# OpenImagingLab/AdaptiveISP

Measured on AMD Instinct MI355X. Metric: ISP+YOLO forward images/sec @1280x720 bs8, higher is better.
Workload: dtype bf16; 1 GPU; batch 8 x 1280x720 fp32 RGB, 5-step ISP schedule ['E', 'CCM', 'NLM', 'Shr', 'T'] (teacher-forced, policy/heads evaluated every step) + YOLOv3 forward @1280x736 bf16 (random-init weights); per_gpu_batch=8, global_batch=8, parallelism=replicas x1

## Files before the change

### adaptiveisp_amd/_lib.py

```python
import ctypes
import os

import numpy as np
import torch

_HERE = os.path.dirname(os.path.abspath(__file__))
LIB_PATH = os.environ.get("ADAISP_LIB") or os.path.join(_HERE, "csrc", "libadaisp.so")

OP_ZERO, OP_EXPOSURE, OP_GAMMA, OP_CCM, OP_SHARPEN, OP_NLM, OP_TONE = -1, 0, 1, 2, 3, 4, 5
OP_CONTRAST, OP_SATPLUS, OP_WNB, OP_WB, OP_USM, OP_SHARPEN_V2, OP_COLOR = 6, 7, 8, 9, 10, 11, 12
MAX_PARAMS = 24
CLIP01 = 1
NLM_EXACT = 2
NLM_SEP_V1 = 4
NO_USM = 8
NLM_TILE32 = 16
ABI_VERSION = 9
UNP_UNPROCESS = 1
UNP_NOISE = 2

EXPORTS = ("adaisp_forward", "adaisp_forward_uniform", "adaisp_process", "adaisp_backward_params", "adaisp_backward_image", "adaisp_backward_image_workspace_bytes", "adaisp_pool64", "adaisp_pool64_backward", "adaisp_demosaic", "adaisp_unprocess", "adaisp_unprocess_bayer", "adaisp_demosaic_rects", "adaisp_demosaic_ex", "adaisp_demosaic_rects_ex", "adaisp_resize_u8", "adaisp_raw_load", "adaisp_raw_correct", "adaisp_export_u8", "adaisp_nlm_general", "adaisp_nlm_general_workspace_bytes", "adaisp_num_params",
           "adaisp_policy_conv", "adaisp_policy_fc1", "adaisp_policy_finish",
           "adaisp_trunk_train_fwd", "adaisp_trunk_train_bwd", "adaisp_trunk_train_workspace_bytes", "adaisp_trunk_train_scratch_bytes",
           "adaisp_critic_planes_fwd", "adaisp_critic_planes_bwd", "adaisp_td_fwd", "adaisp_td_bwd",
           "adaisp_policy_tail_fwd", "adaisp_policy_tail_bwd", "adaisp_image_stats", "adaisp_clip_adam_step", "adaisp_clip_adam_step_dev", "adaisp_heads_fwd", "adaisp_heads_bwd",
           "adaisp_strerror", "adaisp_abi_version")

_lib = None


class AdaispError(RuntimeError):
    pass


def load():
    global _lib
    if _lib is not None:
        return _lib
    if not os.path.exists(LIB_PATH):
# ... 84 lines not shown


def _stream():
    return ctypes.c_void_p(torch.cuda.current_stream().cuda_stream)


def _img_shape(img):
    if img.dim() != 4 or img.shape[1] != 3:
        raise ValueError(f"expected a [B,3,H,W] image, got {tuple(img.shape)}")
    return int(img.shape[0]), int(img.shape[2]), int(img.shape[3])


def image_stats(img):
    L = load()
    img = _dev_f32(img.detach(), "img")
    B = int(img.shape[0])
    buf = torch.empty((B, 2 + 128), dtype=torch.float32, device=img.device)
    with torch.cuda.device(img.device):
        rc = L.adaisp_image_stats(img.data_ptr(), buf.data_ptr(), buf.data_ptr() + 8 * B, B, img.numel() // B, _stream())
    _check(rc, "adaisp_image_stats")
    return buf.view(-1)[:2 * B].view(B, 2)


def process(op, img, params, clip=False, out=None, nlm_exact=False, nlm_v1=False, nlm_tile32=False):
    L = load()
    img = _dev_f32(img, "img")
    B, H, W = _img_shape(img)
    params = _dev_f32(params.reshape(B, -1), "params")
    if out is None:
        out = torch.empty_like(img)
    with torch.cuda.device(img.device):
        rc = L.adaisp_process(int(op), img.data_ptr(), out.data_ptr(), params.data_ptr(), params.shape[1], B, H, W,
                              (CLIP01 if clip else 0) | (NLM_EXACT if nlm_exact else 0) | (NLM_SEP_V1 if nlm_v1 else 0) |
                              (NLM_TILE32 if nlm_tile32 else 0),
                              _stream())
    _check(rc, "adaisp_process")
    _wrote(out)
    return out


def forward(img, op_ids, params, clip=True, pooled=None, out=None, nlm_exact=False, no_usm=False, host_op=None):
    L = load()
    img = _dev_f32(img, "img")
    B, H, W = _img_shape(img)
    params = _dev_f32(params.reshape(B, -1), "params")
    if host_op is None:
        if op_ids.dtype != torch.int32 or not op_ids.is_cuda:
            raise TypeError("op_ids must be an int32 device tensor")
        op_ids = op_ids.contiguous()
    if pooled is not None and (tuple(pooled.shape) != (B, 3, 64, 64) or pooled.dtype != torch.float32 or
                               pooled.device != img.device or not pooled.is_contiguous()):
        raise ValueError(f"pooled must be a contiguous float32 [{B},3,64,64] tensor on {img.device}")
    if out is None:
        out = torch.empty_like(img)
    elif (out.shape != img.shape or out.dtype != torch.float32 or out.device != img.device or not out.is_contiguous()):
        raise ValueError(f"out must be a contiguous float32 {tuple(img.shape)} tensor on {img.device}, got {out.dtype} "
                         f"{tuple(out.shape)} on {out.device}")
    flags = (CLIP01 if clip else 0) | (NLM_EXACT if nlm_exact else 0) | (NO_USM if no_usm else 0)
    with torch.cuda.device(img.device):
        if host_op is not None:
            rc = L.adaisp_forward_uniform(int(host_op), img.data_ptr(), out.data_ptr(),
                                          pooled.data_ptr() if pooled is not None else None, params.data_ptr(),
                                          params.shape[1], B, H, W, flags, _stream())
        else:
            rc = L.adaisp_forward(img.data_ptr(), out.data_ptr(), pooled.data_ptr() if pooled is not None else None,
                                  op_ids.data_ptr(), params.data_ptr(), params.shape[1], B, H, W, flags, _stream())
    _check(rc, "adaisp_forward")
    _wrote(out)
    _wrote(pooled)
    return out


def nlm_general(img, h, search_window_size, patch_size, out=None):
    L = load()
    img = _dev_f32(img, "img")
    B, H, W = _img_shape(img)
    h = _dev_f32(h.reshape(B, -1), "h")
    if out is None:
        out = torch.empty_like(img)
    nbytes = int(L.adaisp_nlm_general_workspace_bytes(B, H, W))
    ws = torch.empty(nbytes // 4, dtype=torch.float32, device=img.device)
# ... 316 lines not shown
```

### adaptiveisp_amd/csrc/isp_nlm.hip

```cpp
#include "isp_filter_math.h"
#ifndef NLM_FMA
#define NLM_FMA 1
#endif
#ifndef NLM_ABL
#define NLM_ABL 0
#endif

namespace adaisp {
namespace {

constexpr int kThreads = 256;
constexpr int TW = 64, TH = 32, RPT = 8;
constexpr int SR = 5, PR = 2;
constexpr int HY = SR + PR;
constexpr int YP = TW + 2 * HY;
constexpr int YROWS = TH + 2 * HY;
constexpr int CP = TW + 2 * SR;
constexpr int CROWS = TH + 2 * SR;
constexpr int NK = RPT + 2 * PR;
constexpr int kYBytes = ((YROWS * YP * 8 + 15) / 16) * 16;
constexpr int kSmemBytes = kYBytes + 3 * CROWS * CP * 4;

typedef float v2f __attribute__((ext_vector_type(2)));

__device__ __forceinline__ v2f pk_sub_bcast_lo(v2f a, v2f b) {
    v2f d;
    asm("v_pk_add_f32 %0, %1, %2 op_sel_hi:[0,1] neg_lo:[0,1] neg_hi:[0,1]" : "=v"(d) : "v"(a), "v"(b));
    return d;
}
__device__ __forceinline__ v2f pk_sub_bcast_hi(v2f a, v2f b) {
    return v2f{a.y, a.y} - b;
}

template <bool GRAD>
__global__ __launch_bounds__(kThreads) void k_nlm(const float* __restrict__ img, float* __restrict__ out,
                                                  const int32_t* __restrict__ ids, int uniform_op,
                                                  const float* __restrict__ params, int pstride, int H, int W,
                                                  const float* __restrict__ grad_out, float* __restrict__ grad_params) {
    extern __shared__ __attribute__((aligned(16))) unsigned char nlm_smem[];
    v2f* ylds2 = reinterpret_cast<v2f*>(nlm_smem);
    float* clds = reinterpret_cast<float*>(nlm_smem + kYBytes);

    const int b = blockIdx.z;
    const int op = ids ? ids[b] : uniform_op;
    if (op != ADAISP_OP_NLM) return;
    const long plane = (long)H * W;
    const float* __restrict__ in = img + (long)b * 3 * plane;
    float* __restrict__ o = out + (long)b * 3 * plane;
    const int x0 = blockIdx.x * TW, y0 = blockIdx.y * TH;
    const int tid = threadIdx.x;
// ... 284 lines not shown
        if (mine && params[(long)b * pstride] > 0.0f) {
#pragma unroll
            for (int r = 0; r < RPT; ++r) {
                const int gy = y0 + rb + r;
                if (gy < H) {
                    const long g = (long)gy * W + gx;
#pragma unroll
                    for (int c = 0; c < 3; ++c) {
                        const float oc = num[c][r] / den[r];
                        if (oc >= 0.0f && oc <= 1.0f) acc += go[g + c * plane] * (ga[c][r] - oc * gb[r]) / den[r];
                    }
                }
            }
        }
        __shared__ float red[4];
#pragma unroll
        for (int off = 32; off > 0; off >>= 1) acc += __shfl_xor(acc, off, 64);
        if ((tid & 63) == 0) red[tid >> 6] = acc;
        __syncthreads();
        if (tid == 0) atomicAdd(grad_params + (long)b * pstride, (red[0] + red[1]) + (red[2] + red[3]));
    }
}

template <int RQ>
__global__ __launch_bounds__(kThreads) void k_nlm_fwd(const float* __restrict__ img, float* __restrict__ out,
                                                      const int32_t* __restrict__ ids, int uniform_op,
                                                      const float* __restrict__ params, int pstride, int H, int W) {
    constexpr int TH = 8 * RQ, HALF = TH / 2;
    constexpr int YROWS = TH + 2 * HY, CROWS = TH + 2 * SR;
    constexpr int Y2ROWS = YROWS - HALF;
    constexpr int B2ROWS = CROWS - HALF;
    __shared__ v2f y2[Y2ROWS * SP];
    __shared__ v2f crg[CROWS * SP];
    __shared__ v2f cb2[B2ROWS * SP];
    const int b = blockIdx.z;
    const int op = ids ? ids[b] : uniform_op;
    if (op != ADAISP_OP_NLM) return;
    const long plane = (long)H * W;
    const float* __restrict__ in = img + (long)b * 3 * plane;
    const int x0 = blockIdx.x * SW, y0 = blockIdx.y * TH;
    const int tid = threadIdx.x;

    float* y2f = reinterpret_cast<float*>(y2);
    float* cb2f = reinterpret_cast<float*>(cb2);
    for (int q0 = tid; q0 < YROWS * SP; q0 += 4 * kThreads) {
        float rr[4], gg4[4], bb4[4];
#pragma unroll
// ... 16 lines not shown
            const int cy = ly - PR;
            if (cy >= 0 && cy < CROWS) {
                crg[cy * SP + lx] = v2f{r, gg};
                if (cy < B2ROWS) cb2f[(cy * SP + lx) * 2] = bb;
                if (cy >= HALF) cb2f[((cy - HALF) * SP + lx) * 2 + 1] = bb;
            }
        }
    }
    __syncthreads();

    const int lane = tid & 63, ty = tid >> 6;
    const int rb = ty * RQ;
    const float hh = fmaxf(params[(long)b * pstride], 0.0f) + 1e-8f;
    const float nc = -1.44269504088896341f / hh;

    v2f yc2[RQ + 2 * PR];
#pragma unroll
    for (int j = 0; j < RQ + 2 * PR; ++j) yc2[j] = y2[(rb + HY - PR + j) * SP + lane + SR];

    v2f nrgA[RQ], nrgB[RQ], nb2[RQ], den2[RQ];
#pragma unroll
    for (int i = 0; i < RQ; ++i) nrgA[i] = nrgB[i] = nb2[i] = den2[i] = v2f{0.0f, 0.0f};

    for (int dx = -SR; dx <= SR; ++dx) {
        for (int dy = -SR; dy <= SR; ++dy) {
            const v2f* ys = y2 + (rb + HY - PR - dy) * SP + lane + SR - dx;
            float c[2 * RQ];
#if NLM_FMA
            v2f dd[RQ + 2 * PR];
#pragma unroll
            for (int j = 0; j < RQ + 2 * PR; ++j) dd[j] = yc2[j] - ys[j * SP];
#pragma unroll
            for (int i = 0; i < RQ; ++i) {
                v2f cc = dd[i + 4] * dd[i + 4];
                cc = __builtin_elementwise_fma(dd[i + 3], dd[i + 3], cc);
                cc = __builtin_elementwise_fma(dd[i + 2], dd[i + 2], cc);
                cc = __builtin_elementwise_fma(dd[i + 1], dd[i + 1], cc);
                cc = __builtin_elementwise_fma(dd[i], dd[i], cc);
                c[2 * i] = cc.x;
                c[2 * i + 1] = cc.y;
            }
#else
            v2f S[RQ + 2 * PR];
#pragma unroll
            for (int j = 0; j < RQ + 2 * PR; ++j) {
                const v2f d = yc2[j] - ys[j * SP];
                S[j] = d * d;
            }
#pragma unroll
            for (int i = 0; i < RQ; ++i) {
                const v2f cc = (((S[i + 4] + S[i + 3]) + S[i + 2]) + S[i + 1]) + S[i];
                c[2 * i] = cc.x;
                c[2 * i + 1] = cc.y;
            }
#endif
            float D[2 * RQ], t1[2 * RQ], t2[2 * RQ], P[2 * RQ];
#if NLM_ABL == 2
#pragma unroll
            for (int i = 0; i < 2 * RQ; ++i) D[i] = c[i];
            if (false)
#endif
            if constexpr (RQ == 4) {
                asm("s_nop 1\n\t"
                    "v_add_f32_dpp %8, %32, %32 wave_shl:1 row_mask:0xf bank_mask:0xf bound_ctrl:0\n\t"
                    "v_add_f32_dpp %9, %33, %33 wave_shl:1 row_mask:0xf bank_mask:0xf bound_ctrl:0\n\t"
                    "v_add_f32_dpp %10, %34, %34 wave_shl:1 row_mask:0xf bank_mask:0xf bound_ctrl:0\n\t"
                    "v_add_f32_dpp %11, %35, %35 wave_shl:1 row_mask:0xf bank_mask:0xf bound_ctrl:0\n\t"
                    "v_add_f32_dpp %12, %36, %36 wave_shl:1 row_mask:0xf bank_mask:0xf bound_ctrl:0\n\t"
                    "v_add_f32_dpp %13, %37, %37 wave_shl:1 row_mask:0xf bank_mask:0xf bound_ctrl:0\n\t"
                    "v_add_f32_dpp %14, %38, %38 wave_shl:1 row_mask:0xf bank_mask:0xf bound_ctrl:0\n\t"
                    "v_add_f32_dpp %15, %39, %39 wave_shl:1 row_mask:0xf bank_mask:0xf bound_ctrl:0\n\t"
                    "v_add_f32_dpp %24, %32, %32 wave_shr:1 row_mask:0xf bank_mask:0xf bound_ctrl:0\n\t"
                    "v_add_f32_dpp %25, %33, %33 wave_shr:1 row_mask:0xf bank_mask:0xf bound_ctrl:0\n\t"
                    "v_add_f32_dpp %26, %34, %34 wave_shr:1 row_mask:0xf bank_mask:0xf bound_ctrl:0\n\t"
                    "v_add_f32_dpp %27, %35, %35 wave_shr:1 row_mask:0xf bank_mask:0xf bound_ctrl:0\n\t"
                    "v_add_f32_dpp %28, %36, %36 wave_shr:1 row_mask:0xf bank_mask:0xf bound_ctrl:0\n\t"
                    "v_add_f32_dpp %29, %37, %37 wave_shr:1 row_mask:0xf bank_mask:0xf bound_ctrl:0\n\t"
                    "v_add_f32_dpp %30, %38, %38 wave_shr:1 row_mask:0xf bank_mask:0xf bound_ctrl:0\n\t"
                    "v_add_f32_dpp %31, %39, %39 wave_shr:1 row_mask:0xf bank_mask:0xf bound_ctrl:0\n\t"
                    "v_add_f32_dpp %16, %8, %32 wave_shl:1 row_mask:0xf bank_mask:0xf bound_ctrl:0\n\t"
                    "v_add_f32_dpp %17, %9, %33 wave_shl:1 row_mask:0xf bank_mask:0xf bound_ctrl:0\n\t"
                    "v_add_f32_dpp %18, %10, %34 wave_shl:1 row_mask:0xf bank_mask:0xf bound_ctrl:0\n\t"
                    "v_add_f32_dpp %19, %11, %35 wave_shl:1 row_mask:0xf bank_mask:0xf bound_ctrl:0\n\t"
                    "v_add_f32_dpp %20, %12, %36 wave_shl:1 row_mask:0xf bank_mask:0xf bound_ctrl:0\n\t"
                    "v_add_f32_dpp %21, %13, %37 wave_shl:1 row_mask:0xf bank_mask:0xf bound_ctrl:0\n\t"
                    "v_add_f32_dpp %22, %14, %38 wave_shl:1 row_mask:0xf bank_mask:0xf bound_ctrl:0\n\t"
                    "v_add_f32_dpp %23, %15, %39 wave_shl:1 row_mask:0xf bank_mask:0xf bound_ctrl:0\n\t"
                    "v_add_f32_dpp %0, %24, %16 wave_shr:1 row_mask:0xf bank_mask:0xf bound_ctrl:0\n\t"
                    "v_add_f32_dpp %1, %25, %17 wave_shr:1 row_mask:0xf bank_mask:0xf bound_ctrl:0\n\t"
                    "v_add_f32_dpp %2, %26, %18 wave_shr:1 row_mask:0xf bank_mask:0xf bound_ctrl:0\n\t"
                    "v_add_f32_dpp %3, %27, %19 wave_shr:1 row_mask:0xf bank_mask:0xf bound_ctrl:0\n\t"
                    "v_add_f32_dpp %4, %28, %20 wave_shr:1 row_mask:0xf bank_mask:0xf bound_ctrl:0\n\t"
                    "v_add_f32_dpp %5, %29, %21 wave_shr:1 row_mask:0xf bank_mask:0xf bound_ctrl:0\n\t"
                    "v_add_f32_dpp %6, %30, %22 wave_shr:1 row_mask:0xf bank_mask:0xf bound_ctrl:0\n\t"
                    "v_add_f32_dpp %7, %31, %23 wave_shr:1 row_mask:0xf bank_mask:0xf bound_ctrl:0"
                    : "=&v"(D[0]), "=&v"(D[1]), "=&v"(D[2]), "=&v"(D[3]), "=&v"(D[4]), "=&v"(D[5]), "=&v"(D[6]), "=&v"(D[7]),
                      "=&v"(t1[0]), "=&v"(t1[1]), "=&v"(t1[2]), "=&v"(t1[3]), "=&v"(t1[4]), "=&v"(t1[5]), "=&v"(t1[6]), "=&v"(t1[7]),
                      "=&v"(t2[0]), "=&v"(t2[1]), "=&v"(t2[2]), "=&v"(t2[3]), "=&v"(t2[4]), "=&v"(t2[5]), "=&v"(t2[6]), "=&v"(t2[7]),
                      "=&v"(P[0]), "=&v"(P[1]), "=&v"(P[2]), "=&v"(P[3]), "=&v"(P[4]), "=&v"(P[5]), "=&v"(P[6]), "=&v"(P[7])
                    : "v"(c[0]), "v"(c[1]), "v"(c[2]), "v"(c[3]), "v"(c[4]), "v"(c[5]), "v"(c[6]), "v"(c[7]));
            } else {
                asm("s_nop 1\n\t"
                    "v_add_f32_dpp %6, %24, %24 wave_shl:1 row_mask:0xf bank_mask:0xf bound_ctrl:0\n\t"
                    "v_add_f32_dpp %7, %25, %25 wave_shl:1 row_mask:0xf bank_mask:0xf bound_ctrl:0\n\t"
                    "v_add_f32_dpp %8, %26, %26 wave_shl:1 row_mask:0xf bank_mask:0xf bound_ctrl:0\n\t"
                    "v_add_f32_dpp %9, %27, %27 wave_shl:1 row_mask:0xf bank_mask:0xf bound_ctrl:0\n\t"
                    "v_add_f32_dpp %10, %28, %28 wave_shl:1 row_mask:0xf bank_mask:0xf bound_ctrl:0\n\t"
                    "v_add_f32_dpp %11, %29, %29 wave_shl:1 row_mask:0xf bank_mask:0xf bound_ctrl:0\n\t"
                    "v_add_f32_dpp %18, %24, %24 wave_shr:1 row_mask:0xf bank_mask:0xf bound_ctrl:0\n\t"
                    "v_add_f32_dpp %19, %25, %25 wave_shr:1 row_mask:0xf bank_mask:0xf bound_ctrl:0\n\t"
                    "v_add_f32_dpp %20, %26, %26 wave_shr:1 row_mask:0xf bank_mask:0xf bound_ctrl:0\n\t"
                    "v_add_f32_dpp %21, %27, %27 wave_shr:1 row_mask:0xf bank_mask:0xf bound_ctrl:0\n\t"
                    "v_add_f32_dpp %22, %28, %28 wave_shr:1 row_mask:0xf bank_mask:0xf bound_ctrl:0\n\t"
                    "v_add_f32_dpp %23, %29, %29 wave_shr:1 row_mask:0xf bank_mask:0xf bound_ctrl:0\n\t"
                    "v_add_f32_dpp %12, %6, %24 wave_shl:1 row_mask:0xf bank_mask:0xf bound_ctrl:0\n\t"
                    "v_add_f32_dpp %13, %7, %25 wave_shl:1 row_mask:0xf bank_mask:0xf bound_ctrl:0\n\t"
                    "v_add_f32_dpp %14, %8, %26 wave_shl:1 row_mask:0xf bank_mask:0xf bound_ctrl:0\n\t"
                    "v_add_f32_dpp %15, %9, %27 wave_shl:1 row_mask:0xf bank_mask:0xf bound_ctrl:0\n\t"
                    "v_add_f32_dpp %16, %10, %28 wave_shl:1 row_mask:0xf bank_mask:0xf bound_ctrl:0\n\t"
                    "v_add_f32_dpp %17, %11, %29 wave_shl:1 row_mask:0xf bank_mask:0xf bound_ctrl:0\n\t"
                    "v_add_f32_dpp %0, %18, %12 wave_shr:1 row_mask:0xf bank_mask:0xf bound_ctrl:0\n\t"
                    "v_add_f32_dpp %1, %19, %13 wave_shr:1 row_mask:0xf bank_mask:0xf bound_ctrl:0\n\t"
                    "v_add_f32_dpp %2, %20, %14 wave_shr:1 row_mask:0xf bank_mask:0xf bound_ctrl:0\n\t"
                    "v_add_f32_dpp %3, %21, %15 wave_shr:1 row_mask:0xf bank_mask:0xf bound_ctrl:0\n\t"
                    "v_add_f32_dpp %4, %22, %16 wave_shr:1 row_mask:0xf bank_mask:0xf bound_ctrl:0\n\t"
                    "v_add_f32_dpp %5, %23, %17 wave_shr:1 row_mask:0xf bank_mask:0xf bound_ctrl:0"
                    : "=&v"(D[0]), "=&v"(D[1]), "=&v"(D[2]), "=&v"(D[3]), "=&v"(D[4]), "=&v"(D[5]),
                      "=&v"(t1[0]), "=&v"(t1[1]), "=&v"(t1[2]), "=&v"(t1[3]), "=&v"(t1[4]), "=&v"(t1[5]),
                      "=&v"(t2[0]), "=&v"(t2[1]), "=&v"(t2[2]), "=&v"(t2[3]), "=&v"(t2[4]), "=&v"(t2[5]),
                      "=&v"(P[0]), "=&v"(P[1]), "=&v"(P[2]), "=&v"(P[3]), "=&v"(P[4]), "=&v"(P[5])
                    : "v"(c[0]), "v"(c[1]), "v"(c[2]), "v"(c[3]), "v"(c[4]), "v"(c[5]));
            }
            const v2f* rg = crg + (rb + SR - dy) * SP + lane + SR - dx;
            const v2f* bl = cb2 + (rb + SR - dy) * SP + lane + SR - dx;
#pragma unroll
            for (int i = 0; i < RQ; ++i) {
#if NLM_ABL == 1
                const v2f wgt = v2f{D[2 * i], D[2 * i + 1]} * nc + 1.0f;
#elif NLM_ABL == 4
                const v2f ex = v2f{D[2 * i], D[2 * i + 1]} * nc;
                const v2f wgt = v2f{__builtin_amdgcn_exp2f(ex.x), __builtin_amdgcn_exp2f(ex.y)};
#else
                const v2f dist = v2f{__builtin_amdgcn_sqrtf(D[2 * i]), __builtin_amdgcn_sqrtf(D[2 * i + 1])};
                const v2f ex = dist * nc;
                const v2f wgt = v2f{__builtin_amdgcn_exp2f(ex.x), __builtin_amdgcn_exp2f(ex.y)};
#endif
#if NLM_ABL == 3
                den2[i] += wgt;
                continue;
#endif
                nrgA[i] = __builtin_elementwise_fma(rg[i * SP], v2f{wgt.x, wgt.x}, nrgA[i]);
                nrgB[i] = __builtin_elementwise_fma(rg[(i + HALF) * SP], v2f{wgt.y, wgt.y}, nrgB[i]);
                nb2[i] = __builtin_elementwise_fma(bl[i * SP], wgt, nb2[i]);
                den2[i] += wgt;
            }
        }
    }

    const int gx = x0 - 2 + lane;
    const bool mine = lane >= 2 && lane < 2 + SW && gx < W;
    float* __restrict__ o = out + (long)b * 3 * plane;
    if (mine) {
#pragma unroll
        for (int i = 0; i < RQ; ++i)
#pragma unroll
            for (int e = 0; e < 2; ++e) {
                const int gy = y0 + rb + i + e * HALF;
                if (gy < H) {
                    const long g = (long)gy * W + gx;
                    const float den = den2[i][e];
                    const v2f n2 = e ? nrgB[i] : nrgA[i];
                    o[g] = clamp01(n2.x / den);
                    o[g + plane] = clamp01(n2.y / den);
                    o[g + 2 * plane] = clamp01(nb2[i][e] / den);
                }
            }
    }
// ... 36 lines not shown
        }
    float* o = out + (long)b * 3 * plane + (long)yy * W + x;
    o[0] = clamp01(n0 / den); o[plane] = clamp01(n1 / den); o[2 * plane] = clamp01(n2 / den);
}

}

hipError_t launch_nlm_general(const float* img, float* out, const float* h, int hstride, float* workspace, int B, int H, int W,
                              int search, int patch, hipStream_t s) {
    const long plane = (long)H * W, total = plane * B;
    hipLaunchKernelGGL(k_nlm_luma, dim3((unsigned)((total + kThreads - 1) / kThreads)), dim3(kThreads), 0, s, img, workspace, plane, total);
    hipLaunchKernelGGL(k_nlm_general, dim3((W + 63) / 64, (H + 3) / 4, B), dim3(kThreads), 0, s, img, workspace, out, h, hstride, H, W,
                       search / 2, patch / 2);
    return hipGetLastError();
}

hipError_t launch_nlm(const Batch& a, hipStream_t s) {
    if (!(a.flags & ADAISP_NLM_EXACT)) {
        dim3 g((a.W + SW - 1) / SW, (a.H + TH - 1) / TH, a.B);
        if (a.flags & ADAISP_NLM_SEP_V1)
            hipLaunchKernelGGL(k_nlm_sep<false>, g, dim3(kThreads), 0, s, a.img, a.out, a.ids, a.uniform_op, a.params,
                               a.pstride, a.H, a.W, static_cast<const float*>(nullptr), static_cast<float*>(nullptr));
        else if (a.flags & ADAISP_NLM_TILE32)
            hipLaunchKernelGGL(k_nlm_fwd<4>, g, dim3(kThreads), 0, s, a.img, a.out, a.ids, a.uniform_op, a.params, a.pstride,
                               a.H, a.W);
        else
            hipLaunchKernelGGL(k_nlm_fwd<3>, dim3(g.x, (a.H + 23) / 24, a.B), dim3(kThreads), 0, s, a.img, a.out, a.ids,
                               a.uniform_op, a.params, a.pstride, a.H, a.W);
        return hipGetLastError();
    }
    dim3 grid((a.W + TW - 1) / TW, (a.H + TH - 1) / TH, a.B);
    static bool configured = false;
    if (!configured) {
        hipError_t e = hipFuncSetAttribute(reinterpret_cast<const void*>(k_nlm<false>),
                                           hipFuncAttributeMaxDynamicSharedMemorySize, kSmemBytes);
        if (e != hipSuccess) return e;
        configured = true;
    }
    hipLaunchKernelGGL(k_nlm<false>, grid, dim3(kThreads), kSmemBytes, s, a.img, a.out, a.ids, a.uniform_op, a.params, a.pstride,
                       a.H, a.W, static_cast<const float*>(nullptr), static_cast<float*>(nullptr));
    return hipGetLastError();
}

hipError_t launch_nlm_backward(const float* img, const float* grad_out, const int32_t* ids, const float* params,
                               int pstride, float* grad_params, int B, int H, int W, unsigned flags, hipStream_t s) {
    if (!(flags & ADAISP_NLM_EXACT)) {
        dim3 g((W + SW - 1) / SW, (H + TH - 1) / TH, B);
        hipLaunchKernelGGL(k_nlm_sep<true>, g, dim3(kThreads), 0, s, img, static_cast<float*>(nullptr), ids, 0, params,
                           pstride, H, W, grad_out, grad_params);
        return hipGetLastError();
    }
// ... 15 lines not shown
```

### include/adaisp.h

```cpp
#ifndef ADAISP_H_
#define ADAISP_H_

#include <stdint.h>

#ifdef __cplusplus
extern "C" {
#endif

#define ADAISP_ABI_VERSION 9

enum adaisp_op {
    ADAISP_OP_ZERO       = -1,
    ADAISP_OP_EXPOSURE   = 0,
    ADAISP_OP_GAMMA      = 1,
    ADAISP_OP_CCM        = 2,
    ADAISP_OP_SHARPEN    = 3,
    ADAISP_OP_NLM        = 4,
    ADAISP_OP_TONE       = 5,
    ADAISP_OP_CONTRAST   = 6,
    ADAISP_OP_SATPLUS    = 7,
    ADAISP_OP_WNB        = 8,
    ADAISP_OP_WB         = 9,
    ADAISP_OP_USM        = 10,
    ADAISP_OP_SHARPEN_V2 = 11,
    ADAISP_OP_COLOR      = 12,
    ADAISP_OP_COUNT      = 13
};

#define ADAISP_MAX_PARAMS 24

#define ADAISP_CLIP01 1u
#define ADAISP_NLM_EXACT 2u
#define ADAISP_NLM_SEP_V1 4u
#define ADAISP_NO_USM 8u
#define ADAISP_NLM_TILE32 16u

#define ADAISP_OK          0
#define ADAISP_EINVAL     -1
#define ADAISP_EOP        -2
#define ADAISP_EALIAS     -3
#define ADAISP_ESHAPE     -4
#define ADAISP_ELAUNCH    -5

int adaisp_forward(const float* img, float* out, float* pooled64_next,
                   const int32_t* filter_id, const float* params, int param_stride,
                   int B, int H, int W, unsigned flags, void* stream);

int adaisp_forward_uniform(int op, const float* img, float* out, float* pooled64_next,
                           const float* params, int param_stride,
                           int B, int H, int W, unsigned flags, void* stream);

int adaisp_process(int op, const float* img, float* out,
                   const float* params, int param_stride,
                   int B, int H, int W, unsigned flags, void* stream);

int adaisp_backward_params(const float* img, const float* grad_out,
                           const int32_t* filter_id, const float* params, int param_stride,
                           float* grad_params,
// ... 284 lines not shown
```

Before: 1975 images/sec.

## Software-pipeline NLM search loop with register sliding window across dy offsets

Refactors the NLM forward kernel's inner search loop into helper functions and adds a pipelined variant, used by default, for the 3-row-per-thread path. As dy advances, the variant slides guide and colour rows through registers, loading only one new row per step, and prefetches the next offset's LDS data before the current compute, with sched_barrier fences between the two. It aims to cut LDS reads and hide LDS latency behind the distance/exp arithmetic. The cost is higher register pressure, which may lower occupancy. The old path stays reachable through a new NLM_PLAIN flag.

Measured after the change: 1993 images/sec, median of 6. Within noise of the previous version (+0.9%).

```diff
diff --git a/adaptiveisp_amd/_lib.py b/adaptiveisp_amd/_lib.py
--- a/adaptiveisp_amd/_lib.py
+++ b/adaptiveisp_amd/_lib.py
@@ -15,6 +15,7 @@
 NLM_SEP_V1 = 4
 NO_USM = 8
 NLM_TILE32 = 16
+NLM_PLAIN = 32
 ABI_VERSION = 9
 UNP_UNPROCESS = 1
 UNP_NOISE = 2
@@ -145,7 +146,7 @@
     return buf.view(-1)[:2 * B].view(B, 2)
 
 
-def process(op, img, params, clip=False, out=None, nlm_exact=False, nlm_v1=False, nlm_tile32=False):
+def process(op, img, params, clip=False, out=None, nlm_exact=False, nlm_v1=False, nlm_tile32=False, nlm_plain=False):
     L = load()
     img = _dev_f32(img, "img")
     B, H, W = _img_shape(img)
@@ -155,14 +156,15 @@
     with torch.cuda.device(img.device):
         rc = L.adaisp_process(int(op), img.data_ptr(), out.data_ptr(), params.data_ptr(), params.shape[1], B, H, W,
                               (CLIP01 if clip else 0) | (NLM_EXACT if nlm_exact else 0) | (NLM_SEP_V1 if nlm_v1 else 0) |
-                              (NLM_TILE32 if nlm_tile32 else 0),
+                              (NLM_TILE32 if nlm_tile32 else 0) | (NLM_PLAIN if nlm_plain else 0),
                               _stream())
     _check(rc, "adaisp_process")
     _wrote(out)
     return out
 
 
-def forward(img, op_ids, params, clip=True, pooled=None, out=None, nlm_exact=False, no_usm=False, host_op=None):
+def forward(img, op_ids, params, clip=True, pooled=None, out=None, nlm_exact=False, no_usm=False, host_op=None,
+            nlm_plain=False):
     L = load()
     img = _dev_f32(img, "img")
     B, H, W = _img_shape(img)
@@ -179,7 +181,8 @@
     elif (out.shape != img.shape or out.dtype != torch.float32 or out.device != img.device or not out.is_contiguous()):
         raise ValueError(f"out must be a contiguous float32 {tuple(img.shape)} tensor on {img.device}, got {out.dtype} "
                          f"{tuple(out.shape)} on {out.device}")
-    flags = (CLIP01 if clip else 0) | (NLM_EXACT if nlm_exact else 0) | (NO_USM if no_usm else 0)
+    flags = ((CLIP01 if clip else 0) | (NLM_EXACT if nlm_exact else 0) | (NO_USM if no_usm else 0) |
+             (NLM_PLAIN if nlm_plain else 0))
     with torch.cuda.device(img.device):
         if host_op is not None:
             rc = L.adaisp_forward_uniform(int(host_op), img.data_ptr(), out.data_ptr(),
diff --git a/adaptiveisp_amd/csrc/isp_nlm.hip b/adaptiveisp_amd/csrc/isp_nlm.hip
--- a/adaptiveisp_amd/csrc/isp_nlm.hip
+++ b/adaptiveisp_amd/csrc/isp_nlm.hip
@@ -26,6 +26,11 @@
 __device__ __forceinline__ v2f pk_sub_bcast_lo(v2f a, v2f b) {
     v2f d;
     asm("v_pk_add_f32 %0, %1, %2 op_sel_hi:[0,1] neg_lo:[0,1] neg_hi:[0,1]" : "=v"(d) : "v"(a), "v"(b));
+    return d;
+}
+__device__ __forceinline__ v2f pk_sub(v2f a, v2f b) {
+    v2f d;
+    asm("v_pk_add_f32 %0, %1, %2 neg_lo:[0,1] neg_hi:[0,1]" : "=v"(d) : "v"(a), "v"(b));
     return d;
 }
 __device__ __forceinline__ v2f pk_sub_bcast_hi(v2f a, v2f b) {
@@ -356,7 +361,146 @@
     }
 }
 
+template <int RQ, class Diff>
+__device__ __forceinline__ void nlm_col_sums(Diff diff, float (&c)[2 * RQ]) {
+#if NLM_FMA
+    v2f dd[RQ + 2 * PR];
+#pragma unroll
+    for (int j = 0; j < RQ + 2 * PR; ++j) dd[j] = diff(j);
+#pragma unroll
+    for (int i = 0; i < RQ; ++i) {
+        v2f cc = dd[i + 4] * dd[i + 4];
+        cc = __builtin_elementwise_fma(dd[i + 3], dd[i + 3], cc);
+        cc = __builtin_elementwise_fma(dd[i + 2], dd[i + 2], cc);
+        cc = __builtin_elementwise_fma(dd[i + 1], dd[i + 1], cc);
+        cc = __builtin_elementwise_fma(dd[i], dd[i], cc);
+        c[2 * i] = cc.x;
+        c[2 * i + 1] = cc.y;
+    }
+#else
+    v2f S[RQ + 2 * PR];
+#pragma unroll
+    for (int j = 0; j < RQ + 2 * PR; ++j) {
+        const v2f d = diff(j);
+        S[j] = d * d;
+    }
+#pragma unroll
+    for (int i = 0; i < RQ; ++i) {
+        const v2f cc = (((S[i + 4] + S[i + 3]) + S[i + 2]) + S[i + 1]) + S[i];
+        c[2 * i] = cc.x;
+        c[2 * i + 1] = cc.y;
+    }
+#endif
+}
+
 template <int RQ>
+__device__ __forceinline__ void nlm_row_sums(const float (&c)[2 * RQ], float (&D)[2 * RQ]) {
+    float t1[2 * RQ], t2[2 * RQ], P[2 * RQ];
+#if NLM_ABL == 2
+#pragma unroll
+    for (int i = 0; i < 2 * RQ; ++i) D[i] = c[i];
+    if (false)
+#endif
+    if constexpr (RQ == 4) {
+        asm("s_nop 1\n\t"
+            "v_add_f32_dpp %8, %32, %32 wave_shl:1 row_mask:0xf bank_mask:0xf bound_ctrl:0\n\t"
+            "v_add_f32_dpp %9, %33, %33 wave_shl:1 row_mask:0xf bank_mask:0xf bound_ctrl:0\n\t"
+            "v_add_f32_dpp %10, %34, %34 wave_shl:1 row_mask:0xf bank_mask:0xf bound_ctrl:0\n\t"
+            "v_add_f32_dpp %11, %35, %35 wave_shl:1 row_mask:0xf bank_mask:0xf bound_ctrl:0\n\t"
+            "v_add_f32_dpp %12, %36, %36 wave_shl:1 row_mask:0xf bank_mask:0xf bound_ctrl:0\n\t"
+            "v_add_f32_dpp %13, %37, %37 wave_shl:1 row_mask:0xf bank_mask:0xf bound_ctrl:0\n\t"
+            "v_add_f32_dpp %14, %38, %38 wave_shl:1 row_mask:0xf bank_mask:0xf bound_ctrl:0\n\t"
+            "v_add_f32_dpp %15, %39, %39 wave_shl:1 row_mask:0xf bank_mask:0xf bound_ctrl:0\n\t"
+            "v_add_f32_dpp %24, %32, %32 wave_shr:1 row_mask:0xf bank_mask:0xf bound_ctrl:0\n\t"
+            "v_add_f32_dpp %25, %33, %33 wave_shr:1 row_mask:0xf bank_mask:0xf bound_ctrl:0\n\t"
+            "v_add_f32_dpp %26, %34, %34 wave_shr:1 row_mask:0xf bank_mask:0xf bound_ctrl:0\n\t"
+            "v_add_f32_dpp %27, %35, %35 wave_shr:1 row_mask:0xf bank_mask:0xf bound_ctrl:0\n\t"
+            "v_add_f32_dpp %28, %36, %36 wave_shr:1 row_mask:0xf bank_mask:0xf bound_ctrl:0\n\t"
+            "v_add_f32_dpp %29, %37, %37 wave_shr:1 row_mask:0xf bank_mask:0xf bound_ctrl:0\n\t"
+            "v_add_f32_dpp %30, %38, %38 wave_shr:1 row_mask:0xf bank_mask:0xf bound_ctrl:0\n\t"
+            "v_add_f32_dpp %31, %39, %39 wave_shr:1 row_mask:0xf bank_mask:0xf bound_ctrl:0\n\t"
+            "v_add_f32_dpp %16, %8, %32 wave_shl:1 row_mask:0xf bank_mask:0xf bound_ctrl:0\n\t"
+            "v_add_f32_dpp %17, %9, %33 wave_shl:1 row_mask:0xf bank_mask:0xf bound_ctrl:0\n\t"
+            "v_add_f32_dpp %18, %10, %34 wave_shl:1 row_mask:0xf bank_mask:0xf bound_ctrl:0\n\t"
+            "v_add_f32_dpp %19, %11, %35 wave_shl:1 row_mask:0xf bank_mask:0xf bound_ctrl:0\n\t"
+            "v_add_f32_dpp %20, %12, %36 wave_shl:1 row_mask:0xf bank_mask:0xf bound_ctrl:0\n\t"
+            "v_add_f32_dpp %21, %13, %37 wave_shl:1 row_mask:0xf bank_mask:0xf bound_ctrl:0\n\t"
+            "v_add_f32_dpp %22, %14, %38 wave_shl:1 row_mask:0xf bank_mask:0xf bound_ctrl:0\n\t"
+            "v_add_f32_dpp %23, %15, %39 wave_shl:1 row_mask:0xf bank_mask:0xf bound_ctrl:0\n\t"
+            "v_add_f32_dpp %0, %24, %16 wave_shr:1 row_mask:0xf bank_mask:0xf bound_ctrl:0\n\t"
+            "v_add_f32_dpp %1, %25, %17 wave_shr:1 row_mask:0xf bank_mask:0xf bound_ctrl:0\n\t"
+            "v_add_f32_dpp %2, %26, %18 wave_shr:1 row_mask:0xf bank_mask:0xf bound_ctrl:0\n\t"
+            "v_add_f32_dpp %3, %27, %19 wave_shr:1 row_mask:0xf bank_mask:0xf bound_ctrl:0\n\t"
+            "v_add_f32_dpp %4, %28, %20 wave_shr:1 row_mask:0xf bank_mask:0xf bound_ctrl:0\n\t"
+            "v_add_f32_dpp %5, %29, %21 wave_shr:1 row_mask:0xf bank_mask:0xf bound_ctrl:0\n\t"
+            "v_add_f32_dpp %6, %30, %22 wave_shr:1 row_mask:0xf bank_mask:0xf bound_ctrl:0\n\t"
+            "v_add_f32_dpp %7, %31, %23 wave_shr:1 row_mask:0xf bank_mask:0xf bound_ctrl:0"
+            : "=&v"(D[0]), "=&v"(D[1]), "=&v"(D[2]), "=&v"(D[3]), "=&v"(D[4]), "=&v"(D[5]), "=&v"(D[6]), "=&v"(D[7]),
+              "=&v"(t1[0]), "=&v"(t1[1]), "=&v"(t1[2]), "=&v"(t1[3]), "=&v"(t1[4]), "=&v"(t1[5]), "=&v"(t1[6]), "=&v"(t1[7]),
+              "=&v"(t2[0]), "=&v"(t2[1]), "=&v"(t2[2]), "=&v"(t2[3]), "=&v"(t2[4]), "=&v"(t2[5]), "=&v"(t2[6]), "=&v"(t2[7]),
+              "=&v"(P[0]), "=&v"(P[1]), "=&v"(P[2]), "=&v"(P[3]), "=&v"(P[4]), "=&v"(P[5]), "=&v"(P[6]), "=&v"(P[7])
+            : "v"(c[0]), "v"(c[1]), "v"(c[2]), "v"(c[3]), "v"(c[4]), "v"(c[5]), "v"(c[6]), "v"(c[7]));
+    } else {
+        asm("s_nop 1\n\t"
+            "v_add_f32_dpp %6, %24, %24 wave_shl:1 row_mask:0xf bank_mask:0xf bound_ctrl:0\n\t"
+            "v_add_f32_dpp %7, %25, %25 wave_shl:1 row_mask:0xf bank_mask:0xf bound_ctrl:0\n\t"
+            "v_add_f32_dpp %8, %26, %26 wave_shl:1 row_mask:0xf bank_mask:0xf bound_ctrl:0\n\t"
+            "v_add_f32_dpp %9, %27, %27 wave_shl:1 row_mask:0xf bank_mask:0xf bound_ctrl:0\n\t"
+            "v_add_f32_dpp %10, %28, %28 wave_shl:1 row_mask:0xf bank_mask:0xf bound_ctrl:0\n\t"
+            "v_add_f32_dpp %11, %29, %29 wave_shl:1 row_mask:0xf bank_mask:0xf bound_ctrl:0\n\t"
+            "v_add_f32_dpp %18, %24, %24 wave_shr:1 row_mask:0xf bank_mask:0xf bound_ctrl:0\n\t"
+            "v_add_f32_dpp %19, %25, %25 wave_shr:1 row_mask:0xf bank_mask:0xf bound_ctrl:0\n\t"
+            "v_add_f32_dpp %20, %26, %26 wave_shr:1 row_mask:0xf bank_mask:0xf bound_ctrl:0\n\t"
+            "v_add_f32_dpp %21, %27, %27 wave_shr:1 row_mask:0xf bank_mask:0xf bound_ctrl:0\n\t"
+            "v_add_f32_dpp %22, %28, %28 wave_shr:1 row_mask:0xf bank_mask:0xf bound_ctrl:0\n\t"
+            "v_add_f32_dpp %23, %29, %29 wave_shr:1 row_mask:0xf bank_mask:0xf bound_ctrl:0\n\t"
+            "v_add_f32_dpp %12, %6, %24 wave_shl:1 row_mask:0xf bank_mask:0xf bound_ctrl:0\n\t"
+            "v_add_f32_dpp %13, %7, %25 wave_shl:1 row_mask:0xf bank_mask:0xf bound_ctrl:0\n\t"
+            "v_add_f32_dpp %14, %8, %26 wave_shl:1 row_mask:0xf bank_mask:0xf bound_ctrl:0\n\t"
+            "v_add_f32_dpp %15, %9, %27 wave_shl:1 row_mask:0xf bank_mask:0xf bound_ctrl:0\n\t"
+            "v_add_f32_dpp %16, %10, %28 wave_shl:1 row_mask:0xf bank_mask:0xf bound_ctrl:0\n\t"
+            "v_add_f32_dpp %17, %11, %29 wave_shl:1 row_mask:0xf bank_mask:0xf bound_ctrl:0\n\t"
+            "v_add_f32_dpp %0, %18, %12 wave_shr:1 row_mask:0xf bank_mask:0xf bound_ctrl:0\n\t"
+            "v_add_f32_dpp %1, %19, %13 wave_shr:1 row_mask:0xf bank_mask:0xf bound_ctrl:0\n\t"
+            "v_add_f32_dpp %2, %20, %14 wave_shr:1 row_mask:0xf bank_mask:0xf bound_ctrl:0\n\t"
+            "v_add_f32_dpp %3, %21, %15 wave_shr:1 row_mask:0xf bank_mask:0xf bound_ctrl:0\n\t"
+            "v_add_f32_dpp %4, %22, %16 wave_shr:1 row_mask:0xf bank_mask:0xf bound_ctrl:0\n\t"
+            "v_add_f32_dpp %5, %23, %17 wave_shr:1 row_mask:0xf bank_mask:0xf bound_ctrl:0"
+            : "=&v"(D[0]), "=&v"(D[1]), "=&v"(D[2]), "=&v"(D[3]), "=&v"(D[4]), "=&v"(D[5]),
+              "=&v"(t1[0]), "=&v"(t1[1]), "=&v"(t1[2]), "=&v"(t1[3]), "=&v"(t1[4]), "=&v"(t1[5]),
+              "=&v"(t2[0]), "=&v"(t2[1]), "=&v"(t2[2]), "=&v"(t2[3]), "=&v"(t2[4]), "=&v"(t2[5]),
+              "=&v"(P[0]), "=&v"(P[1]), "=&v"(P[2]), "=&v"(P[3]), "=&v"(P[4]), "=&v"(P[5])
+            : "v"(c[0]), "v"(c[1]), "v"(c[2]), "v"(c[3]), "v"(c[4]), "v"(c[5]));
+    }
+}
+
+template <int RQ, class RgA, class RgB, class Bl>
+__device__ __forceinline__ void nlm_weigh(const float (&D)[2 * RQ], float nc, RgA rgA, RgB rgB, Bl bl, v2f (&nrgA)[RQ],
+                                          v2f (&nrgB)[RQ], v2f (&nb2)[RQ], v2f (&den2)[RQ]) {
+#pragma unroll
+    for (int i = 0; i < RQ; ++i) {
+#if NLM_ABL == 1
+        const v2f wgt = v2f{D[2 * i], D[2 * i + 1]} * nc + 1.0f;
+#elif NLM_ABL == 4
+        const v2f ex = v2f{D[2 * i], D[2 * i + 1]} * nc;
+        const v2f wgt = v2f{__builtin_amdgcn_exp2f(ex.x), __builtin_amdgcn_exp2f(ex.y)};
+#else
+        const v2f dist = v2f{__builtin_amdgcn_sqrtf(D[2 * i]), __builtin_amdgcn_sqrtf(D[2 * i + 1])};
+        const v2f ex = dist * nc;
+        const v2f wgt = v2f{__builtin_amdgcn_exp2f(ex.x), __builtin_amdgcn_exp2f(ex.y)};
+#endif
+#if NLM_ABL == 3
+        den2[i] += wgt;
+        continue;
+#endif
+        nrgA[i] = __builtin_elementwise_fma(rgA(i), v2f{wgt.x, wgt.x}, nrgA[i]);
+        nrgB[i] = __builtin_elementwise_fma(rgB(i), v2f{wgt.y, wgt.y}, nrgB[i]);
+        nb2[i] = __builtin_elementwise_fma(bl(i), wgt, nb2[i]);
+        den2[i] += wgt;
+    }
+}
+
+template <int RQ, bool PIPE>
 __global__ __launch_bounds__(kThreads) void k_nlm_fwd(const float* __restrict__ img, float* __restrict__ out,
                                                       const int32_t* __restrict__ ids, int uniform_op,
                                                       const float* __restrict__ params, int pstride, int H, int W) {
@@ -419,137 +563,69 @@
 #pragma unroll
     for (int i = 0; i < RQ; ++i) nrgA[i] = nrgB[i] = nb2[i] = den2[i] = v2f{0.0f, 0.0f};
 
-    for (int dx = -SR; dx <= SR; ++dx) {
-        for (int dy = -SR; dy <= SR; ++dy) {
-            const v2f* ys = y2 + (rb + HY - PR - dy) * SP + lane + SR - dx;
-            float c[2 * RQ];
-#if NLM_FMA
-            v2f dd[RQ + 2 * PR];
-#pragma unroll
-            for (int j = 0; j < RQ + 2 * PR; ++j) dd[j] = yc2[j] - ys[j * SP];
-#pragma unroll
-            for (int i = 0; i < RQ; ++i) {
-                v2f cc = dd[i + 4] * dd[i + 4];
-                cc = __builtin_elementwise_fma(dd[i + 3], dd[i + 3], cc);
-                cc = __builtin_elementwise_fma(dd[i + 2], dd[i + 2], cc);
-                cc = __builtin_elementwise_fma(dd[i + 1], dd[i + 1], cc);
-                cc = __builtin_elementwise_fma(dd[i], dd[i], cc);
-                c[2 * i] = cc.x;
-                c[2 * i + 1] = cc.y;
-            }
-#else
-            v2f S[RQ + 2 * PR];
-#pragma unroll
-            for (int j = 0; j < RQ + 2 * PR; ++j) {
-                const v2f d = yc2[j] - ys[j * SP];
-                S[j] = d * d;
-            }
-#pragma unroll
-            for (int i = 0; i < RQ; ++i) {
-                const v2f cc = (((S[i + 4] + S[i + 3]) + S[i + 2]) + S[i + 1]) + S[i];
-                c[2 * i] = cc.x;
-                c[2 * i + 1] = cc.y;
-            }
-#endif
-            float D[2 * RQ], t1[2 * RQ], t2[2 * RQ], P[2 * RQ];
-#if NLM_ABL == 2
-#pragma unroll
-            for (int i = 0; i < 2 * RQ; ++i) D[i] = c[i];
-            if (false)
-#endif
-            if constexpr (RQ == 4) {
-                asm("s_nop 1\n\t"
-                    "v_add_f32_dpp %8, %32, %32 wave_shl:1 row_mask:0xf bank_mask:0xf bound_ctrl:0\n\t"
-                    "v_add_f32_dpp %9, %33, %33 wave_shl:1 row_mask:0xf bank_mask:0xf bound_ctrl:0\n\t"
-                    "v_add_f32_dpp %10, %34, %34 wave_shl:1 row_mask:0xf bank_mask:0xf bound_ctrl:0\n\t"
-                    "v_add_f32_dpp %11, %35, %35 wave_shl:1 row_mask:0xf bank_mask:0xf bound_ctrl:0\n\t"
-                    "v_add_f32_dpp %12, %36, %36 wave_shl:1 row_mask:0xf bank_mask:0xf bound_ctrl:0\n\t"
-                    "v_add_f32_dpp %13, %37, %37 wave_shl:1 row_mask:0xf bank_mask:0xf bound_ctrl:0\n\t"
-                    "v_add_f32_dpp %14, %38, %38 wave_shl:1 row_mask:0xf bank_mask:0xf bound_ctrl:0\n\t"
-                    "v_add_f32_dpp %15, %39, %39 wave_shl:1 row_mask:0xf bank_mask:0xf bound_ctrl:0\n\t"
-                    "v_add_f32_dpp %24, %32, %32 wave_shr:1 row_mask:0xf bank_mask:0xf bound_ctrl:0\n\t"
-                    "v_add_f32_dpp %25, %33, %33 wave_shr:1 row_mask:0xf bank_mask:0xf bound_ctrl:0\n\t"
-                    "v_add_f32_dpp %26, %34, %34 wave_shr:1 row_mask:0xf bank_mask:0xf bound_ctrl:0\n\t"
-                    "v_add_f32_dpp %27, %35, %35 wave_shr:1 row_mask:0xf bank_mask:0xf bound_ctrl:0\n\t"
-                    "v_add_f32_dpp %28, %36, %36 wave_shr:1 row_mask:0xf bank_mask:0xf bound_ctrl:0\n\t"
-                    "v_add_f32_dpp %29, %37, %37 wave_shr:1 row_mask:0xf bank_mask:0xf bound_ctrl:0\n\t"
-                    "v_add_f32_dpp %30, %38, %38 wave_shr:1 row_mask:0xf bank_mask:0xf bound_ctrl:0\n\t"
-                    "v_add_f32_dpp %31, %39, %39 wave_shr:1 row_mask:0xf bank_mask:0xf bound_ctrl:0\n\t"
-                    "v_add_f32_dpp %16, %8, %32 wave_shl:1 row_mask:0xf bank_mask:0xf bound_ctrl:0\n\t"
-                    "v_add_f32_dpp %17, %9, %33 wave_shl:1 row_mask:0xf bank_mask:0xf bound_ctrl:0\n\t"
-                    "v_add_f32_dpp %18, %10, %34 wave_shl:1 row_mask:0xf bank_mask:0xf bound_ctrl:0\n\t"
-                    "v_add_f32_dpp %19, %11, %35 wave_shl:1 row_mask:0xf bank_mask:0xf bound_ctrl:0\n\t"
-                    "v_add_f32_dpp %20, %12, %36 wave_shl:1 row_mask:0xf bank_mask:0xf bound_ctrl:0\n\t"
-                    "v_add_f32_dpp %21, %13, %37 wave_shl:1 row_mask:0xf bank_mask:0xf bound_ctrl:0\n\t"
-                    "v_add_f32_dpp %22, %14, %38 wave_shl:1 row_mask:0xf bank_mask:0xf bound_ctrl:0\n\t"
-                    "v_add_f32_dpp %23, %15, %39 wave_shl:1 row_mask:0xf bank_mask:0xf bound_ctrl:0\n\t"
-                    "v_add_f32_dpp %0, %24, %16 wave_shr:1 row_mask:0xf bank_mask:0xf bound_ctrl:0\n\t"
-                    "v_add_f32_dpp %1, %25, %17 wave_shr:1 row_mask:0xf bank_mask:0xf bound_ctrl:0\n\t"
-                    "v_add_f32_dpp %2, %26, %18 wave_shr:1 row_mask:0xf bank_mask:0xf bound_ctrl:0\n\t"
-                    "v_add_f32_dpp %3, %27, %19 wave_shr:1 row_mask:0xf bank_mask:0xf bound_ctrl:0\n\t"
-                    "v_add_f32_dpp %4, %28, %20 wave_shr:1 row_mask:0xf bank_mask:0xf bound_ctrl:0\n\t"
-                    "v_add_f32_dpp %5, %29, %21 wave_shr:1 row_mask:0xf bank_mask:0xf bound_ctrl:0\n\t"
-                    "v_add_f32_dpp %6, %30, %22 wave_shr:1 row_mask:0xf bank_mask:0xf bound_ctrl:0\n\t"
-                    "v_add_f32_dpp %7, %31, %23 wave_shr:1 row_mask:0xf bank_mask:0xf bound_ctrl:0"
-                    : "=&v"(D[0]), "=&v"(D[1]), "=&v"(D[2]), "=&v"(D[3]), "=&v"(D[4]), "=&v"(D[5]), "=&v"(D[6]), "=&v"(D[7]),
-                      "=&v"(t1[0]), "=&v"(t1[1]), "=&v"(t1[2]), "=&v"(t1[3]), "=&v"(t1[4]), "=&v"(t1[5]), "=&v"(t1[6]), "=&v"(t1[7]),
-                      "=&v"(t2[0]), "=&v"(t2[1]), "=&v"(t2[2]), "=&v"(t2[3]), "=&v"(t2[4]), "=&v"(t2[5]), "=&v"(t2[6]), "=&v"(t2[7]),
-                      "=&v"(P[0]), "=&v"(P[1]), "=&v"(P[2]), "=&v"(P[3]), "=&v"(P[4]), "=&v"(P[5]), "=&v"(P[6]), "=&v"(P[7])
-                    : "v"(c[0]), "v"(c[1]), "v"(c[2]), "v"(c[3]), "v"(c[4]), "v"(c[5]), "v"(c[6]), "v"(c[7]));
-            } else {
-                asm("s_nop 1\n\t"
-                    "v_add_f32_dpp %6, %24, %24 wave_shl:1 row_mask:0xf bank_mask:0xf bound_ctrl:0\n\t"
-                    "v_add_f32_dpp %7, %25, %25 wave_shl:1 row_mask:0xf bank_mask:0xf bound_ctrl:0\n\t"
-                    "v_add_f32_dpp %8, %26, %26 wave_shl:1 row_mask:0xf bank_mask:0xf bound_ctrl:0\n\t"
-                    "v_add_f32_dpp %9, %27, %27 wave_shl:1 row_mask:0xf bank_mask:0xf bound_ctrl:0\n\t"
-                    "v_add_f32_dpp %10, %28, %28 wave_shl:1 row_mask:0xf bank_mask:0xf bound_ctrl:0\n\t"
-                    "v_add_f32_dpp %11, %29, %29 wave_shl:1 row_mask:0xf bank_mask:0xf bound_ctrl:0\n\t"
-                    "v_add_f32_dpp %18, %24, %24 wave_shr:1 row_mask:0xf bank_mask:0xf bound_ctrl:0\n\t"
-                    "v_add_f32_dpp %19, %25, %25 wave_shr:1 row_mask:0xf bank_mask:0xf bound_ctrl:0\n\t"
-                    "v_add_f32_dpp %20, %26, %26 wave_shr:1 row_mask:0xf bank_mask:0xf bound_ctrl:0\n\t"
-                    "v_add_f32_dpp %21, %27, %27 wave_shr:1 row_mask:0xf bank_mask:0xf bound_ctrl:0\n\t"
-                    "v_add_f32_dpp %22, %28, %28 wave_shr:1 row_mask:0xf bank_mask:0xf bound_ctrl:0\n\t"
-                    "v_add_f32_dpp %23, %29, %29 wave_shr:1 row_mask:0xf bank_mask:0xf bound_ctrl:0\n\t"
-                    "v_add_f32_dpp %12, %6, %24 wave_shl:1 row_mask:0xf bank_mask:0xf bound_ctrl:0\n\t"
-                    "v_add_f32_dpp %13, %7, %25 wave_shl:1 row_mask:0xf bank_mask:0xf bound_ctrl:0\n\t"
-                    "v_add_f32_dpp %14, %8, %26 wave_shl:1 row_mask:0xf bank_mask:0xf bound_ctrl:0\n\t"
-                    "v_add_f32_dpp %15, %9, %27 wave_shl:1 row_mask:0xf bank_mask:0xf bound_ctrl:0\n\t"
-                    "v_add_f32_dpp %16, %10, %28 wave_shl:1 row_mask:0xf bank_mask:0xf bound_ctrl:0\n\t"
-                    "v_add_f32_dpp %17, %11, %29 wave_shl:1 row_mask:0xf bank_mask:0xf bound_ctrl:0\n\t"
-                    "v_add_f32_dpp %0, %18, %12 wave_shr:1 row_mask:0xf bank_mask:0xf bound_ctrl:0\n\t"
-                    "v_add_f32_dpp %1, %19, %13 wave_shr:1 row_mask:0xf bank_mask:0xf bound_ctrl:0\n\t"
-                    "v_add_f32_dpp %2, %20, %14 wave_shr:1 row_mask:0xf bank_mask:0xf bound_ctrl:0\n\t"
-                    "v_add_f32_dpp %3, %21, %15 wave_shr:1 row_mask:0xf bank_mask:0xf bound_ctrl:0\n\t"
-                    "v_add_f32_dpp %4, %22, %16 wave_shr:1 row_mask:0xf bank_mask:0xf bound_ctrl:0\n\t"
-                    "v_add_f32_dpp %5, %23, %17 wave_shr:1 row_mask:0xf bank_mask:0xf bound_ctrl:0"
-                    : "=&v"(D[0]), "=&v"(D[1]), "=&v"(D[2]), "=&v"(D[3]), "=&v"(D[4]), "=&v"(D[5]),
-                      "=&v"(t1[0]), "=&v"(t1[1]), "=&v"(t1[2]), "=&v"(t1[3]), "=&v"(t1[4]), "=&v"(t1[5]),
-                      "=&v"(t2[0]), "=&v"(t2[1]), "=&v"(t2[2]), "=&v"(t2[3]), "=&v"(t2[4]), "=&v"(t2[5]),
-                      "=&v"(P[0]), "=&v"(P[1]), "=&v"(P[2]), "=&v"(P[3]), "=&v"(P[4]), "=&v"(P[5])
-                    : "v"(c[0]), "v"(c[1]), "v"(c[2]), "v"(c[3]), "v"(c[4]), "v"(c[5]));
-            }
-            const v2f* rg = crg + (rb + SR - dy) * SP + lane + SR - dx;
-            const v2f* bl = cb2 + (rb + SR - dy) * SP + lane + SR - dx;
-#pragma unroll
-            for (int i = 0; i < RQ; ++i) {
-#if NLM_ABL == 1
-                const v2f wgt = v2f{D[2 * i], D[2 * i + 1]} * nc + 1.0f;
-#elif NLM_ABL == 4
-                const v2f ex = v2f{D[2 * i], D[2 * i + 1]} * nc;
-                const v2f wgt = v2f{__builtin_amdgcn_exp2f(ex.x), __builtin_amdgcn_exp2f(ex.y)};
-#else
-                const v2f dist = v2f{__builtin_amdgcn_sqrtf(D[2 * i]), __builtin_amdgcn_sqrtf(D[2 * i + 1])};
-                const v2f ex = dist * nc;
-                const v2f wgt = v2f{__builtin_amdgcn_exp2f(ex.x), __builtin_amdgcn_exp2f(ex.y)};
-#endif
-#if NLM_ABL == 3
-                den2[i] += wgt;
-                continue;
-#endif
-                nrgA[i] = __builtin_elementwise_fma(rg[i * SP], v2f{wgt.x, wgt.x}, nrgA[i]);
-                nrgB[i] = __builtin_elementwise_fma(rg[(i + HALF) * SP], v2f{wgt.y, wgt.y}, nrgB[i]);
-                nb2[i] = __builtin_elementwise_fma(bl[i * SP], wgt, nb2[i]);
-                den2[i] += wgt;
+    constexpr int NL = RQ + 2 * PR;
+    if constexpr (!PIPE) {
+        for (int dx = -SR; dx <= SR; ++dx) {
+            for (int dy = -SR; dy <= SR; ++dy) {
+                const v2f* ys = y2 + (rb + HY - PR - dy) * SP + lane + SR - dx;
+                float c[2 * RQ], D[2 * RQ];
+                nlm_col_sums<RQ>([&](int j) { return yc2[j] - ys[j * SP]; }, c);
+                nlm_row_sums<RQ>(c, D);
+                const v2f* rg = crg + (rb + SR - dy) * SP + lane + SR - dx;
+                const v2f* bl = cb2 + (rb + SR - dy) * SP + lane + SR - dx;
+                nlm_weigh<RQ>(D, nc, [&](int i) { return rg[i * SP]; }, [&](int i) { return rg[(i + HALF) * SP]; },
+                              [&](int i) { return bl[i * SP]; }, nrgA, nrgB, nb2, den2);
+            }
+        }
+    } else {
+        const v2f* ys0 = y2 + rb * SP + lane + SR;
+        const v2f* rg0 = crg + rb * SP + lane + SR;
+        const v2f* bl0 = cb2 + rb * SP + lane + SR;
+        v2f sh[NL], a[RQ], bq[RQ], bb[RQ];
+#pragma unroll
+        for (int j = 0; j < NL; ++j) sh[j] = ys0[(2 * SR + j) * SP + SR];
+#pragma unroll
+        for (int i = 0; i < RQ; ++i) {
+            a[i] = rg0[(2 * SR + i) * SP + SR];
+            bq[i] = rg0[(2 * SR + i + HALF) * SP + SR];
+            bb[i] = bl0[(2 * SR + i) * SP + SR];
+        }
+        for (int dx = -SR; dx <= SR; ++dx) {
+            const int dxn = min(dx + 1, SR);
+#pragma unroll
+            for (int dy = -SR; dy <= SR; ++dy) {
+                v2f nsh[NL], na[RQ], nbq[RQ], nbb[RQ];
+                if (dy < SR) {
+                    const int t = SR - (dy + 1);
+                    nsh[0] = ys0[t * SP - dx];
+                    na[0] = rg0[t * SP - dx];
+                    nbq[0] = rg0[(t + HALF) * SP - dx];
+                    nbb[0] = bl0[t * SP - dx];
+#pragma unroll
+                    for (int j = 1; j < NL; ++j) nsh[j] = sh[j - 1];
+#pragma unroll
+                    for (int i = 1; i < RQ; ++i) { na[i] = a[i - 1]; nbq[i] = bq[i - 1]; nbb[i] = bb[i - 1]; }
+                } else {
+#pragma unroll
+                    for (int j = 0; j < NL; ++j) nsh[j] = ys0[(2 * SR + j) * SP - dxn];
+#pragma unroll
+                    for (int i = 0; i < RQ; ++i) {
+                        na[i] = rg0[(2 * SR + i) * SP - dxn];
+                        nbq[i] = rg0[(2 * SR + i + HALF) * SP - dxn];
+                        nbb[i] = bl0[(2 * SR + i) * SP - dxn];
+                    }
+                }
+                __builtin_amdgcn_sched_barrier(0);
+                float c[2 * RQ], D[2 * RQ];
+                nlm_col_sums<RQ>([&](int j) { return pk_sub(yc2[j], sh[j]); }, c);
+                nlm_row_sums<RQ>(c, D);
+                nlm_weigh<RQ>(D, nc, [&](int i) { return a[i]; }, [&](int i) { return bq[i]; }, [&](int i) { return bb[i]; },
+                              nrgA, nrgB, nb2, den2);
+                __builtin_amdgcn_sched_barrier(0);
+#pragma unroll
+                for (int j = 0; j < NL; ++j) sh[j] = nsh[j];
+#pragma unroll
+                for (int i = 0; i < RQ; ++i) { a[i] = na[i]; bq[i] = nbq[i]; bb[i] = nbb[i]; }
             }
         }
     }
@@ -632,11 +708,14 @@
             hipLaunchKernelGGL(k_nlm_sep<false>, g, dim3(kThreads), 0, s, a.img, a.out, a.ids, a.uniform_op, a.params,
                                a.pstride, a.H, a.W, static_cast<const float*>(nullptr), static_cast<float*>(nullptr));
         else if (a.flags & ADAISP_NLM_TILE32)
-            hipLaunchKernelGGL(k_nlm_fwd<4>, g, dim3(kThreads), 0, s, a.img, a.out, a.ids, a.uniform_op, a.params, a.pstride,
-                               a.H, a.W);
+            hipLaunchKernelGGL((k_nlm_fwd<4, false>), g, dim3(kThreads), 0, s, a.img, a.out, a.ids, a.uniform_op, a.params,
+                               a.pstride, a.H, a.W);
+        else if (a.flags & ADAISP_NLM_PLAIN)
+            hipLaunchKernelGGL((k_nlm_fwd<3, false>), dim3(g.x, (a.H + 23) / 24, a.B), dim3(kThreads), 0, s, a.img, a.out,
+                               a.ids, a.uniform_op, a.params, a.pstride, a.H, a.W);
         else
-            hipLaunchKernelGGL(k_nlm_fwd<3>, dim3(g.x, (a.H + 23) / 24, a.B), dim3(kThreads), 0, s, a.img, a.out, a.ids,
-                               a.uniform_op, a.params, a.pstride, a.H, a.W);
+            hipLaunchKernelGGL((k_nlm_fwd<3, true>), dim3(g.x, (a.H + 23) / 24, a.B), dim3(kThreads), 0, s, a.img, a.out,
+                               a.ids, a.uniform_op, a.params, a.pstride, a.H, a.W);
         return hipGetLastError();
     }
     dim3 grid((a.W + TW - 1) / TW, (a.H + TH - 1) / TH, a.B);
diff --git a/include/adaisp.h b/include/adaisp.h
--- a/include/adaisp.h
+++ b/include/adaisp.h
@@ -34,6 +34,7 @@
 #define ADAISP_NLM_SEP_V1 4u
 #define ADAISP_NO_USM 8u
 #define ADAISP_NLM_TILE32 16u
+#define ADAISP_NLM_PLAIN 32u
 
 #define ADAISP_OK          0
 #define ADAISP_EINVAL     -1
```
